# viniciusvidal2/slam-sensor-fusion

Hardware: AMD Instinct MI355X
Metric: scans_per_s_200k_scan_vs_10M_map (higher is better)
Workload: dtype f32 points / f64 accumulation

## Files before the change

### slam_sensor_fusion_amd/csrc/sf_icp.hip

```cpp
#include "sf_common.hpp"
#include "sf_nn.hpp"
#include "sf_tile.hpp"
#include "sf_order.hpp"
#include "sf_p2p.hpp"

#include <cfloat>
#include <cstdlib>
#include <cmath>
#include <vector>
#include <mutex>
#include <string>

namespace {

constexpr int BLK = 256;
constexpr int NREC_P2P = 17;
constexpr int NREC_PLANE = 30;
constexpr int REC_STRIDE = 32;

struct IcpState {
    double T[16];
    double rec[REC_STRIDE];
    double fitness, rmse, prev_fitness, prev_rmse;
    float last_error, err_pending;
// ... 799 lines not shown
        for (int k = 0; k < 12; ++k) P.T[k] = (float)st[b].T[k];
        return P;
    }
    __device__ __forceinline__ Point load(uint32_t o) const { return Point{x[o], y[o], z[o]}; }
    __device__ __forceinline__ uint32_t full_key(const Pose &P, const Point &p) const
    {
        const float qx = fmaf(P.T[0], p.x, fmaf(P.T[1], p.y, fmaf(P.T[2], p.z, P.T[3])));
        const float qy = fmaf(P.T[4], p.x, fmaf(P.T[5], p.y, fmaf(P.T[6], p.z, P.T[7])));
        const float qz = fmaf(P.T[8], p.x, fmaf(P.T[9], p.y, fmaf(P.T[10], p.z, P.T[11])));
        if (!(isfinite(qx) && isfinite(qy) && isfinite(qz))) return TILE_KEY_NONE;
        const int cx = (int)fminf(fmaxf(floorf((qx - g.org[0]) * g.inv_h), 0.0f), (float)(g.dim[0] - 1));
        const int cy = (int)fminf(fmaxf(floorf((qy - g.org[1]) * g.inv_h), 0.0f), (float)(g.dim[1] - 1));
        const int cz = (int)fminf(fmaxf(floorf((qz - g.org[2]) * g.inv_h), 0.0f), (float)(g.dim[2] - 1));
        return sf::tile_of_cell(tl, cx, cy, cz);
    }
    __device__ __forceinline__ uint32_t key(const Pose &P, const Point &p) const { return (full_key(P, p) >> (sf::ORD_KEY_BITS * digit)) & (uint32_t)(sf::ORD_BINS - 1); }
};

__global__ __launch_bounds__(sf::ORD_BLK) void k_order_hist_tile(sf::OrderSrc s, TileKeyFn kf, uint16_t *__restrict__ keys, uint32_t *__restrict__ counts)
{
    sf::order_hist_body(s, kf, keys, counts);
}

__global__ __launch_bounds__(256) void k_tile_keys(TileKeyFn kf, int64_t total, uint32_t *__restrict__ tkey)
{
    const int64_t o = (int64_t)blockIdx.x * 256 + threadIdx.x;
    if (o >= total) return;
    const int b = (int)(o / kf.n);
    tkey[o] = kf.full_key(kf.prepare(b), kf.load((uint32_t)o));
}

__global__ __launch_bounds__(256) void k_tile_starts(const uint32_t *__restrict__ tkey, int n, int batch, int ntiles, uint32_t *__restrict__ seg)
{
    const int64_t i = (int64_t)blockIdx.x * 256 + threadIdx.x;
    if (i >= (int64_t)(ntiles + 1) * batch) return;
    const uint32_t t = (uint32_t)(i / batch);
    const int b = (int)(i % batch);
    const uint32_t *k = tkey + (size_t)b * n;
    int lo = 0, hi = n;
    while (lo < hi) {
        const int mid = (lo + hi) >> 1;
        if (k[mid] < t) lo = mid + 1; else hi = mid;
    }
    seg[i] = (uint32_t)lo;
}

constexpr int TILE_STATS = 8;
#ifdef SF_PHASE_TRACE
__device__ unsigned long long g_tile_trace[sf::PH_SHARDS * sf::PH_SLOTS];
#define TT_MARK(i) do { if (wv == 0) { const unsigned long long n_ = __builtin_amdgcn_s_memtime(); tt_acc[i] += (unsigned)(n_ - tt_t); tt_t = n_; } } while (0)
#else
#define TT_MARK(i) do { } while (0)
#endif

template <int MODE>
__global__ __launch_bounds__(sf::TILE_BLK) void k_tile_search(SfGrid g, sf::SfTiles tl, const float *__restrict__ X0x, const float *__restrict__ X0y, const float *__restrict__ X0z,
                                                              int n, int batch, const IcpState *__restrict__ st, float thr, const uint32_t *__restrict__ seg,
                                                              float4 *__restrict__ qcache, int64_t cache_n, int reuse, unsigned long long *__restrict__ stats)
{
    const int per = ((int)gridDim.x) >> 3;
    const int tile = ((int)blockIdx.x & 7) * per + ((int)blockIdx.x >> 3);
    if (tile >= tl.ntiles) return;
    __shared__ sf::TileLds lds;
    __shared__ double Tm[sf::TILE_SCANS][12];
    __shared__ float mot[sf::TILE_SCANS];
    __shared__ int live[sf::TILE_SCANS];
    __shared__ uint32_t pre[sf::TILE_SCANS + 1], gofs[sf::TILE_SCANS];
    __shared__ unsigned int cnt[4];
    const int tid = (int)threadIdx.x, lane = tid & 63, wv = tid >> 6;
    const sf::TileRegion R = sf::tile_region(g, tl, (uint32_t)tile);
#ifdef SF_PHASE_TRACE
    unsigned tt_acc[8] = {0, 0, 0, 0, 0, 0, 0, 0};
    unsigned long long tt_t = __builtin_amdgcn_s_memtime();
#endif
    bool staged = false, fits = false;
    if (tid < 4) cnt[tid] = 0;
    float *ecache = reinterpret_cast<float *>(qcache + (size_t)cache_n);
    SfWindow nowin;
    nowin.kind = 0;
    for (int b0 = 0; b0 < batch; b0 += sf::TILE_SCANS) {
        __syncthreads();
        if (wv == 0) {
            const int b = b0 + lane;
            uint32_t s0 = 0, len = 0;
            if (b < batch && !st[b].done) {
                s0 = seg[(size_t)tile * batch + b];
                len = seg[(size_t)(tile + 1) * batch + b] - s0;
            }
            uint32_t v = len;
#pragma unroll
            for (int o = 1; o < 64; o <<= 1) {
                const uint32_t t = (uint32_t)__shfl_up((int)v, o);
                if (lane >= o) v += t;
            }
            pre[lane + 1] = v;
            if (lane == 0) pre[0] = 0;
            gofs[lane] = (uint32_t)((size_t)b * n + s0);
        }
        for (int i = tid; i < sf::TILE_SCANS * 12; i += sf::TILE_BLK) {
            const int b = b0 + i / 12;
            Tm[i / 12][i % 12] = b < batch ? st[b].T[i % 12] : 0.0;
        }
        if (tid < sf::TILE_SCANS) {
            const int b = b0 + tid;
            mot[tid] = b < batch ? (float)st[b].motion : 0.0f;
            live[tid] = (b < batch && reuse && st[b].cache_live != 0) ? 1 : 0;
        }
        __syncthreads();
        TT_MARK(0);
        const uint32_t total = pre[sf::TILE_SCANS];
        if (total == 0) continue;
        if (!staged) {
            fits = sf::tile_stage(g, R, &lds);
            staged = true;
            if (!fits && tid == 0 && stats) atomicAdd(&stats[4], 1ull);
        }
        TT_MARK(1);
        for (uint32_t i = (uint32_t)tid; i < total; i += sf::TILE_BLK) {
            int bl = 0;
#pragma unroll
            for (int step = 32; step > 0; step >>= 1) bl += (pre[bl + step] <= i) ? step : 0;
            const size_t o = (size_t)gofs[bl] + (size_t)(i - pre[bl]);
            const bool cache_live = live[bl] != 0;
            float4 c1 = make_float4(0.f, 0.f, 0.f, 0.f), c2 = c1;
            float e = 0.0f;
            if (cache_live) {
                c1 = qcache[o];
                if (MODE == 2) { c2 = qcache[(size_t)cache_n + o]; e = c2.w; }
                else e = ecache[o];
            }
            const double x0 = X0x[o], y0 = X0y[o], z0 = X0z[o];
            const double *T = Tm[bl];
            const double sx = T[0] * x0 + T[1] * y0 + T[2] * z0 + T[3];
            const double sy = T[4] * x0 + T[5] * y0 + T[6] * z0 + T[7];
            const double sz = T[8] * x0 + T[9] * y0 + T[10] * z0 + T[11];
            const float qx = (float)sx, qy = (float)sy, qz = (float)sz;
            const float m_now = mot[bl];
            sf::NNHit chit, seed;
            float4 tn;
            bool need = reuse_certificate(true, qx, qy, qz, thr, m_now, e, c1, c2, chit, tn, seed);
            if (!need) {
                if (!cache_live) {
                    if (MODE == 2) qcache[(size_t)cache_n + o] = make_float4(0.f, 0.f, 0.f, 0.f);
                    else ecache[o] = 0.0f;
                }
                continue;
            }
            sf::NNHit hit;
            hit.d2 = sf::search_start(thr);
            hit.j = -1;
            hit.px = hit.py = hit.pz = 0.0f;
            hit.lb2 = 3.0e38f;
            bool walk = g.n > 0;
            {
                const float ox = fmaxf(fmaxf(g.org[0] - qx, qx - (g.org[0] + (float)g.dim[0] * g.h)), 0.0f);
                const float oy = fmaxf(fmaxf(g.org[1] - qy, qy - (g.org[1] + (float)g.dim[1] * g.h)), 0.0f);
                const float oz = fmaxf(fmaxf(g.org[2] - qz, qz - (g.org[2] + (float)g.dim[2] * g.h)), 0.0f);
                const float gap = fmaxf(sqrtf(ox * ox + oy * oy + oz * oz) * 0.9995f - 1.0e-3f, 0.0f);
                if (gap * gap > thr) { hit.lb2 = gap * gap; walk = false; }
            }
            if (walk) {
                const sf::QueryGeo G = sf::query_geo(g, qx, qy, qz);
                int ring_from = 1;
                if (fits && sf::tile_serves(g, R, G)) {
                    bool more;
                    const sf::TileHit th = sf::tile_search(g, R, &lds, G, qx, qy, qz, thr, seed.d2, seed.j, &more);
                    hit.d2 = th.d2; hit.j = th.j; hit.lb2 = th.lb2;
                    if (th.loc >= 0) { const float4 p = lds.pts[th.loc]; hit.px = p.x; hit.py = p.y; hit.pz = p.z; }
                    else if (th.j >= 0) { hit.px = seed.px; hit.py = seed.py; hit.pz = seed.pz; }
                    ring_from = more ? 2 : 0;
                    if (stats) atomicAdd(&cnt[more ? 3 : 1], 1u);
                } else {
                    if (seed.j >= 0 && seed.d2 < thr) { hit.d2 = seed.d2; hit.j = seed.j; hit.px = seed.px; hit.py = seed.py; hit.pz = seed.pz; }
                    if (stats) atomicAdd(&cnt[2], 1u);
                }
                if (ring_from) {
                    sf::nn_rings<false>(g, nowin, qx, qy, qz, ring_from, hit);
                    hit.lb2 = 0.0f;
                }
            }
            if (stats) atomicAdd(&cnt[0], 1u);
            float4 nrm = make_float4(0.f, 0.f, 0.f, 0.f);
            if (MODE == 2 && hit.j >= 0) nrm = g.nrm[hit.j];
            const float en = fmaxf(sqrtf(hit.lb2) * 0.9999f + m_now * 0.999998f - 1.0e-6f, 1.0e-30f);
            qcache[o] = make_float4(hit.px, hit.py, hit.pz, __int_as_float(hit.j));
            if (MODE == 2) qcache[(size_t)cache_n + o] = make_float4(nrm.x, nrm.y, nrm.z, en);
            else ecache[o] = en;
        }
    }
    TT_MARK(2);
    __syncthreads();
    TT_MARK(3);
    if (stats && tid < 4 && cnt[tid]) atomicAdd(&stats[tid], (unsigned long long)cnt[tid]);
#ifdef SF_PHASE_TRACE
    if (tid == 0) {
        tt_acc[7] = 1;
        for (int i = 0; i < 8; ++i) atomicAdd(&g_tile_trace[(size_t)(blockIdx.x & (sf::PH_SHARDS - 1)) * sf::PH_SLOTS + i], (unsigned long long)tt_acc[i]);
    }
#endif
}

template <int MODE, int Q>
__global__ __launch_bounds__(BLK) void k_red_cached(const float *__restrict__ X0x, const float *__restrict__ X0y, const float *__restrict__ X0z, int n,
                                                    const IcpState *__restrict__ st, float thr, double *__restrict__ partials, int nblocks, const float4 *__restrict__ qcache,
                                                    int64_t cache_n)
{
    constexpr int NREC = MODE == 2 ? NREC_PLANE : NREC_P2P;
    const int L = blockIdx.y * gridDim.x + blockIdx.x;
    const int kk = L >> 3;
    const int b = kk % (int)gridDim.y;
    const int bx = (L & 7) * ((int)gridDim.x >> 3) + kk / (int)gridDim.y;
    if (bx >= nblocks) return;
    const IcpState *S = st + b;
    if (S->done) return;
    __shared__ double stage[BLK / 64][32];
    const int wv = threadIdx.x >> 6, lane = threadIdx.x & 63;
    LanePair P[Q];
#pragma unroll
    for (int u = 0; u < Q; ++u) {
        const int slot = bx * (BLK * Q) + u * BLK + (int)threadIdx.x;
        const QueryIn q = query_in<MODE, false>(X0x, X0y, X0z, n, b, S, 0.0f, 0.0f, nullptr, qcache, cache_n, true, slot, n);
        sf::NNHit hit;
// ... 1431 lines not shown
    int64_t fused_redone = 0;
    bool inject_timeout = false;
    int64_t fused_launches = 0;
    IcpState *h_pin = nullptr;
    size_t h_pin_cap = 0;
    bool use_graph = false;
    hipGraphExec_t graph_exec = nullptr;
    int64_t graph_captures = 0, graph_replays = 0;
    struct GraphKey {
        int mode = -1, iters = -1, batch = -1, window = -1, ordered = -1, reuse = -1, robust_kind = -1;
        int64_t n = -1;
        const void *map = nullptr;
        uint64_t map_generation = 0, epochs = 0;
        float max_corr = 0, accept = 0, eps = 0;
        double robust_k = 0;
        bool operator==(const GraphKey &o) const
        {
            return mode == o.mode && iters == o.iters && batch == o.batch && window == o.window && ordered == o.ordered && reuse == o.reuse && n == o.n && map == o.map &&
                   map_generation == o.map_generation && epochs == o.epochs && max_corr == o.max_corr && accept == o.accept && eps == o.eps &&
                   robust_kind == o.robust_kind && robust_k == o.robust_k;
        }
    } graph_key;
    struct Lane {
        sf::DevBuf X, qcache, Xq, qkeys, qkeys2, qidx, qidx2, corr, state, d_inits, partials, fz_state, fz_part, fz_cnt, fz_ids, fz_all, qtkey, tseg, tile_stats;
        hipGraphExec_t graph_exec = nullptr;
        GraphKey graph_key;
        std::vector<double> inits_uploaded;
        uint32_t d_inits_epoch = 0xffffffffu;
    } other;
    struct SrcSet {
        sf::DevBuf X0, X0r, stage, d_boxes, d_box_parts, n_dev;
        int64_t n = 0, n_cap = 0, plane = 0;
        int batch = 0, nblocks = 0, nblocks_nn = 0, qpl = 1;
        bool have_source = false, n_on_device = false;
    } other_src;
    int src_set = 0;
    hipEvent_t src_used[2] = {nullptr, nullptr}, src_ready = nullptr;
    bool src_used_rec[2] = {false, false};
    bool src_ahead = false;
    hipEvent_t started[2] = {nullptr, nullptr};
    bool started_rec[2] = {false, false};
    hipEvent_t unmarked_ev = nullptr;
    bool src_unmarked_use = false;
    struct LaneMeta {
        bool valid = false;
        int batch = 0, mode = 0;
        std::vector<double> inits;
// ... 16 lines not shown
    bool profiling = false;
    std::vector<hipEvent_t> ev;
    size_t ev_used = 0;
    int64_t prof_launches = 0;
    double prof_ms = 0;
    std::vector<float> prof_each;
    std::vector<int> ev_kind;
    std::vector<float> prof_phase[SF_PROF_KINDS];
    sf::DevBuf nn_stats;
    int freeze = 1;
    FreezeParams fz_prm{8.0f, 2.0e-5f, 3.0e-4f, 3};
    int fz_from = 5;
    bool fz_from_auto = true;
    int fz_fetches = 0;
    int fz_step = 0;
    sf::DevBuf fz_state, fz_part, fz_cnt, fz_ids, fz_all;
    int64_t nn_stats_used = 0;
    static constexpr int64_t NN_STATS_CAP = 1024;
    int robust_kind = SF_ROBUST_NONE;
    double robust_k = 0.0;
    int tile_mode = 0;
    bool tile_on = false;
    sf::SfTiles tiles{};
    sf::DevBuf qtkey, tseg, tile_stats;
};

namespace {

float *soa(sf::DevBuf &b, int64_t total, int axis) { return b.as<float>() + (size_t)axis * (size_t)total; }
const float *src(sf_icp *icp, int axis)
{
    if (icp->shard) return soa(icp->Xq, icp->own_total, axis);
    return soa(icp->ordered ? icp->Xq : icp->X0, icp->plane, axis);
}

int fused_capacity(sf_icp *icp, int mode, bool robust = false);

bool robust_on(const sf_icp *icp, int mode) { return mode == SF_ICP_P2PLANE && icp->robust_kind != SF_ROBUST_NONE; }
RobustArg robust_arg(const sf_icp *icp) { return RobustArg{icp->robust_kind, icp->robust_k}; }

constexpr int64_t ORDER_AUTO_MIN_QUERIES = 300000;

int order_key_shift(const SfGrid &g)
{
    const uint64_t ny_pad = ((uint64_t)g.dim[1] + ORDER_YBLK - 1) / ORDER_YBLK * ORDER_YBLK;
    const uint64_t ncell = (uint64_t)g.dim[0] * ny_pad * (uint64_t)g.dim[2];
    int cbits = 0;
// ... 33 lines not shown
        tc[0] = t2[0]; tc[1] = t2[1]; tc[2] = t2[2];
    }
    if (!fits_tables(tc)) return false;
    sf::SfTiles tl;
    int64_t nt = 1;
    for (int a = 0; a < 3; ++a) {
        tl.tc[a] = tc[a];
        tl.nt[a] = (g.dim[a] + tc[a] - 1) / tc[a];
        nt *= tl.nt[a];
    }
    if (nt >= (int64_t)TILE_KEY_NONE) return false;
    tl.ntiles = (int)nt;
    *out = tl;
    return true;
}

bool tile_wanted(const sf_icp *icp, int mode)
{
    if (icp->tile_mode == 0 || robust_on(icp, mode) || icp->shard || icp->map->window.kind != 0 || (mode != SF_ICP_P2PLANE && mode != SF_ICP_O3D_P2P)) return false;
    if (icp->qpl == 1) return false;
    return icp->tile_mode == 2 || icp->n * icp->batch >= TILE_AUTO_MIN_QUERIES;
}

bool tile_launch(const sf_icp *icp, int k) { return icp->tile_on && (!icp->reuse || k < VERIFY_FROM_SEARCH); }

constexpr int ORDER_LUT_BINS = (1 << ORDER_LUT_LOG2) + 1;
int order_lut_prepare(sf_icp *icp)
{
    if (!icp->order_lut_on || !icp->map || !icp->map->built) return SF_OK;
    const SfGrid &g = icp->map->grid;
    if (g.n <= 0 || (icp->order_lut.p && icp->order_lut_gen == icp->map->generation)) return SF_OK;
    const uint64_t ny_pad = ((uint64_t)g.dim[1] + ORDER_YBLK - 1) / ORDER_YBLK * ORDER_YBLK;
    const uint64_t span = (uint64_t)g.dim[0] * ny_pad * (uint64_t)g.dim[2];
    int cbits = 0;
    while (cbits < 63 && (1ull << cbits) < span) ++cbits;
    icp->order_lut_shift = std::max(0, cbits - ORDER_LUT_LOG2);
    const int nbins = (int)(span >> icp->order_lut_shift) + 1;
    SF_TRY(icp->order_lut.reserve(sizeof(uint32_t) * (size_t)ORDER_LUT_BINS + sizeof(uint16_t) * (size_t)ORDER_LUT_BINS));
    uint32_t *hist = icp->order_lut.as<uint32_t>();
    uint16_t *lut = reinterpret_cast<uint16_t *>(hist + ORDER_LUT_BINS);
    hipStream_t st = icp->ctx->stream;
    SF_HIP(hipMemsetAsync(hist, 0, sizeof(uint32_t) * (size_t)ORDER_LUT_BINS, st));
    hipLaunchKernelGGL(k_order_lut_hist, dim3(nblk(g.n)), dim3(256), 0, st, g, icp->order_lut_shift, hist);
    hipLaunchKernelGGL(k_order_lut_make, dim3(1), dim3(1024), 0, st, hist, nbins, (uint32_t)g.n, lut);
    SF_HIP(hipGetLastError());
    icp->order_lut_gen = icp->map->generation;
    return SF_OK;
// ... 54 lines not shown
            hipLaunchKernelGGL(sf::k_order_scan, dim3((unsigned)nseg), dim3(sf::ORD_BINS), 0, s, counts, src2.tiles);
            hipLaunchKernelGGL(k_order_scatter, grid, blk, 0, s, src2, keys, counts, ordered);
        }
    } else {
        hipLaunchKernelGGL(k_order_hist, grid, blk, 0, s, src, kf, keys, counts);
        hipLaunchKernelGGL(sf::k_order_scan, dim3((unsigned)nseg), dim3(sf::ORD_BINS), 0, s, counts, src.tiles);
        hipLaunchKernelGGL(k_order_scatter, grid, blk, 0, s, src, keys, counts, ordered);
    }
    const int64_t qplane = seg_off ? total : icp->plane;
    if (seg_off) {
        hipLaunchKernelGGL(k_order_gather, dim3(nblk(total, GATHER_TILE)), dim3(256), 0, s, icp->X0r.as<float4>(), ordered, total, 0, 0, 0, soa(icp->Xq, qplane, 0),
                           soa(icp->Xq, qplane, 1), soa(icp->Xq, qplane, 2));
    } else {
        const int gt = (int)std::max<int64_t>(1, sf::div_up(icp->n, GATHER_TILE));
        hipLaunchKernelGGL(k_order_gather, dim3(sf::order_grid(gt, nseg)), dim3(256), 0, s, icp->X0r.as<float4>(), ordered, total, (int)icp->n, gt, nseg,
                           soa(icp->Xq, qplane, 0), soa(icp->Xq, qplane, 1), soa(icp->Xq, qplane, 2));
    }
    if (icp->tile_on) {
        TileKeyFn tk;
        tk.g = g; tk.tl = icp->tiles;
        tk.x = soa(icp->Xq, qplane, 0); tk.y = soa(icp->Xq, qplane, 1); tk.z = soa(icp->Xq, qplane, 2);
        tk.st = kf.st; tk.n = (int)icp->n; tk.digit = 0;
        const int64_t rows = (int64_t)icp->tiles.ntiles + 1;
        SF_TRY(icp->qtkey.reserve(sizeof(uint32_t) * cap));
        SF_TRY(icp->tseg.reserve(sizeof(uint32_t) * (size_t)rows * (size_t)nseg));
        SF_TRY(icp->tile_stats.reserve(sizeof(unsigned long long) * TILE_STATS));
        SF_HIP(hipMemsetAsync(icp->tile_stats.p, 0, sizeof(unsigned long long) * TILE_STATS, s));
        hipLaunchKernelGGL(k_tile_keys, dim3(nblk(total)), dim3(256), 0, s, tk, total, icp->qtkey.as<uint32_t>());
        hipLaunchKernelGGL(k_tile_starts, dim3(nblk(rows * nseg)), dim3(256), 0, s, icp->qtkey.as<uint32_t>(), (int)icp->n, nseg, icp->tiles.ntiles, icp->tseg.as<uint32_t>());
    }
    SF_HIP(hipGetLastError());
    return SF_OK;
}

int order_queries(sf_icp *icp, int mode)
{
    const int64_t total = icp->n * icp->batch;
    const bool want = icp->order == SF_ORDER_CELL || (icp->order == SF_ORDER_AUTO && total >= ORDER_AUTO_MIN_QUERIES);
    icp->ordered = false;
    icp->tile_on = false;
    if (!want || total == 0 || icp->map->grid.n == 0 || icp->n_on_device) return SF_OK;
    icp->tile_on = tile_wanted(icp, mode) && tile_plan(icp->map->grid, &icp->tiles);
    SF_TRY(run_order_sort(icp, icp->batch, icp->n, total, nullptr, nullptr));
    icp->ordered = true;
    return SF_OK;
}

void raw_swap(sf::DevBuf &a, sf::DevBuf &b)
{
    std::swap(a.p, b.p);
    std::swap(a.cap, b.cap);
    std::swap(a.epoch, b.epoch);
// ... 150 lines not shown

void prof_collect(sf_icp *icp)
{
    for (size_t k = 0; k + 1 < icp->ev_used; k += 2) {
        float ms = 0;
        if (hipEventElapsedTime(&ms, icp->ev[k], icp->ev[k + 1]) != hipSuccess) continue;
        const int kind = k / 2 < icp->ev_kind.size() ? icp->ev_kind[k / 2] : SF_PROF_NN;
        if (kind == SF_PROF_NN) { icp->prof_ms += ms; icp->prof_launches += 1; icp->prof_each.push_back(ms); }
        else if (kind > 0 && kind < SF_PROF_KINDS) icp->prof_phase[kind].push_back(ms);
    }
    icp->ev_used = 0;
}

sf_icp::GraphKey graph_key_now(const sf_icp *icp, int mode)
{
    sf_icp::GraphKey k;
    k.mode = mode; k.iters = icp->prm.num_iters; k.batch = icp->batch; k.window = icp->map->window.kind; k.ordered = (int)icp->ordered | ((int)icp->tile_on << 1); k.reuse = (int)icp->reuse | (icp->freeze << 1) | (icp->fz_from << 3);
    k.n = (mode == SF_ICP_REF_CPP && icp->batch == 1) ? -icp->n_cap : icp->n;
    k.map = (const void *)icp->map;
    k.map_generation = icp->map->generation;
    k.robust_kind = robust_on(icp, mode) ? icp->robust_kind : SF_ROBUST_NONE; k.robust_k = robust_on(icp, mode) ? icp->robust_k : 0.0;
    k.max_corr = icp->prm.max_corr; k.accept = icp->prm.accept; k.eps = icp->prm.eps + icp->fz_prm.guard_scale * 1.0e-3f + icp->fz_prm.guard_min + icp->fz_prm.guard_max + (float)icp->fz_prm.max_tries;
    const sf::DevBuf *bufs[] = {&icp->X0, &icp->X0r, &icp->X, &icp->Xq, &icp->qcache, &icp->corr, &icp->state, &icp->partials, &icp->d_box, &icp->d_boxes, &icp->n_dev,
                                &icp->map->pts4, &icp->map->nrm4, &icp->map->cell_start, &icp->map->d_window, &icp->fz_state, &icp->fz_part, &icp->fz_cnt, &icp->fz_ids, &icp->fz_all, &icp->tseg, &icp->tile_stats};
    k.epochs = (uint64_t)icp->plane;
    for (const sf::DevBuf *b : bufs) k.epochs = (k.epochs * 1000003ull + b->epoch) * 1000003ull + (uint64_t)(uintptr_t)b->p;
    return k;
}

float o3d_thr(const sf_icp *icp) { return (float)((double)icp->prm.max_corr * (double)icp->prm.max_corr); }

template <int MODE>
void launch_nn_red(sf_icp *icp, bool sharded = false, bool one_per_lane = false)
{
    sf_map *m = icp->map;
    const int nb = sharded ? (one_per_lane ? icp->own_nblocks * icp->qpl : icp->own_nblocks) : (one_per_lane ? icp->nblocks : icp->nblocks_nn);
    const dim3 grid((unsigned)((nb + 7) & ~7), (unsigned)icp->batch), blk(BLK);
    const float *x = src(icp, 0), *y = src(icp, 1), *z = src(icp, 2);
    const IcpState *st = icp->state.as<IcpState>();
    double *part = icp->partials.as<double>();
    const float thr = o3d_thr(icp);
    hipStream_t s = icp->ctx->stream;
    ProfScope ps(icp);
    uint32_t *stats = nullptr;
    if (icp->profiling && icp->nn_stats.p && icp->nn_stats_used < sf_icp::NN_STATS_CAP) stats = icp->nn_stats.as<uint32_t>() + 2 * NN_STATS_SHARDS * icp->nn_stats_used++;
    const bool win = m->window.kind != 0;
    if (MODE == 2 && robust_on(icp, MODE)) {
// ... 5 lines not shown
        if (win && sharded) { if (q1) SF_LAUNCH_NNRED_ROB(true, true, 1); else SF_LAUNCH_NNRED_ROB(true, true, SF_WIDE_QPL); }
        else if (win) { if (q1) SF_LAUNCH_NNRED_ROB(true, false, 1); else SF_LAUNCH_NNRED_ROB(true, false, SF_WIDE_QPL); }
        else if (sharded) { if (q1) SF_LAUNCH_NNRED_ROB(false, true, 1); else SF_LAUNCH_NNRED_ROB(false, true, SF_WIDE_QPL); }
        else { if (q1) SF_LAUNCH_NNRED_ROB(false, false, 1); else SF_LAUNCH_NNRED_ROB(false, false, SF_WIDE_QPL); }
#undef SF_LAUNCH_NNRED_ROB
        return;
    }
#define SF_LAUNCH_NNRED_Q(W, S, QQ)                                                                                                                              \
    hipLaunchKernelGGL((k_nn_red<MODE, W, S, QQ>), grid, blk, 0, s, m->grid, m->window, x, y, z, (int)icp->n, st, thr, icp->xlo, icp->xhi, part, nb, \
                       icp->own_off.as<uint32_t>(), icp->reuse ? icp->qcache.as<float4>() : nullptr, icp->cache_n, stats)
#define SF_LAUNCH_NNRED(W, S)                                  \
    do {                                                       \
        if (icp->qpl == 1 || one_per_lane) SF_LAUNCH_NNRED_Q(W, S, 1); \
        else SF_LAUNCH_NNRED_Q(W, S, SF_WIDE_QPL);             \
    } while (0)
    if (win && sharded) SF_LAUNCH_NNRED(true, true);
    else if (win) SF_LAUNCH_NNRED(true, false);
    else if (sharded) SF_LAUNCH_NNRED(false, true);
    else SF_LAUNCH_NNRED(false, false);
#undef SF_LAUNCH_NNRED_Q
#undef SF_LAUNCH_NNRED
}

template <int MODE>
void launch_tile_search(sf_icp *icp, bool one_per_lane)
{
    sf_map *m = icp->map;
    const int nb = one_per_lane ? icp->nblocks : icp->nblocks_nn;
    const float *x = src(icp, 0), *y = src(icp, 1), *z = src(icp, 2);
    const IcpState *st = icp->state.as<IcpState>();
    const float thr = o3d_thr(icp);
    hipStream_t s = icp->ctx->stream;
    ProfScope ps(icp);
    unsigned long long *stats = icp->profiling ? icp->tile_stats.as<unsigned long long>() : nullptr;
    if (icp->profiling && icp->nn_stats.p && icp->nn_stats_used < sf_icp::NN_STATS_CAP) icp->nn_stats_used++;
    const unsigned tgrid = (unsigned)((icp->tiles.ntiles + 7) & ~7);
    hipLaunchKernelGGL((k_tile_search<MODE>), dim3(tgrid), dim3(sf::TILE_BLK), 0, s, m->grid, icp->tiles, x, y, z, (int)icp->n, icp->batch, st, thr, icp->tseg.as<uint32_t>(),
                       icp->qcache.as<float4>(), icp->cache_n, (int)icp->reuse, stats);
    const dim3 grid((unsigned)((nb + 7) & ~7), (unsigned)icp->batch), blk(BLK);
    if (icp->qpl == 1 || one_per_lane)
        hipLaunchKernelGGL((k_red_cached<MODE, 1>), grid, blk, 0, s, x, y, z, (int)icp->n, st, thr, icp->partials.as<double>(), nb, icp->qcache.as<float4>(), icp->cache_n);
    else
        hipLaunchKernelGGL((k_red_cached<MODE, SF_WIDE_QPL>), grid, blk, 0, s, x, y, z, (int)icp->n, st, thr, icp->partials.as<double>(), nb, icp->qcache.as<float4>(), icp->cache_n);
}

bool freeze_on(const sf_icp *icp, int mode)
{
    const int64_t queries = icp->shard ? icp->own_total : icp->n * icp->batch;
    const bool wanted = icp->freeze == 2 || (icp->freeze == 1 && queries >= FREEZE_AUTO_MIN_QUERIES);
    return mode == SF_ICP_P2PLANE && wanted && !robust_on(icp, mode) && icp->reuse && icp->qpl == SF_WIDE_QPL && icp->map->window.kind == 0 && icp->prm.num_iters > icp->fz_from + 1 &&
           icp->fz_from >= VERIFY_FROM_SEARCH;
}

int freeze_alloc(sf_icp *icp)
{
    const size_t rows = (size_t)icp->batch * (size_t)std::max(icp->nblocks_nn, icp->shard ? icp->own_nblocks : 0);
    SF_TRY(icp->fz_state.reserve(sizeof(FreezeState) * (size_t)icp->batch));
    SF_TRY(icp->fz_part.reserve(sizeof(double) * FZ_NMOM * rows));
    SF_TRY(icp->fz_cnt.reserve(sizeof(uint32_t) * rows));
    SF_TRY(icp->fz_ids.reserve(sizeof(uint16_t) * FZ_CAP * rows));
    SF_TRY(icp->fz_all.reserve(sizeof(uint32_t) * FZ_CAP * rows));
// ... 706 lines not shown
}

extern "C" int sf_icp_test_inject_barrier_timeout(sf_icp *icp)
{
    SF_CHECK(icp, SF_ERR_INVALID, "icp is NULL");
    icp->inject_timeout = true;
    return SF_OK;
}

extern "C" int sf_icp_use_graph(sf_icp *icp, int on)
{
    SF_CHECK(icp, SF_ERR_INVALID, "icp is NULL");
    icp->use_graph = on != 0;
    return SF_OK;
}

namespace {
void lane_flip(sf_icp *icp)
{
    sf_icp::Lane &o = icp->other;
    raw_swap(icp->X, o.X); raw_swap(icp->qcache, o.qcache); raw_swap(icp->Xq, o.Xq); raw_swap(icp->qkeys, o.qkeys); raw_swap(icp->qkeys2, o.qkeys2);
    raw_swap(icp->qidx, o.qidx); raw_swap(icp->qidx2, o.qidx2); raw_swap(icp->corr, o.corr); raw_swap(icp->state, o.state); raw_swap(icp->d_inits, o.d_inits);
    raw_swap(icp->partials, o.partials); raw_swap(icp->fz_state, o.fz_state); raw_swap(icp->fz_part, o.fz_part); raw_swap(icp->fz_cnt, o.fz_cnt);
    raw_swap(icp->fz_ids, o.fz_ids); raw_swap(icp->fz_all, o.fz_all); raw_swap(icp->qtkey, o.qtkey); raw_swap(icp->tseg, o.tseg); raw_swap(icp->tile_stats, o.tile_stats);
    std::swap(icp->graph_exec, o.graph_exec);
    std::swap(icp->graph_key, o.graph_key);
    std::swap(icp->inits_uploaded, o.inits_uploaded);
    std::swap(icp->d_inits_epoch, o.d_inits_epoch);
    std::swap(icp->meta, icp->other_meta);
    icp->lane ^= 1;
}

int lane_reserve(sf_icp *icp)
{
    const int batch = std::max(icp->batch, 1);
    SF_TRY(icp->state.reserve(sizeof(IcpState) * (size_t)batch));
    SF_TRY(icp->d_inits.reserve(sizeof(double) * 16 * (size_t)batch));
    SF_TRY(icp->partials.reserve(sizeof(double) * (size_t)REC_STRIDE * (size_t)std::max(icp->nblocks, 1) * (size_t)batch));
    return SF_OK;
}

struct LaneScope {
    sf_icp *icp;
    hipStream_t main = nullptr;
    bool piped = false;
    int rc = SF_OK;
    LaneScope(sf_icp *i, bool allowed) : icp(i)
// ... 550 lines not shown
```

### slam_sensor_fusion_amd/csrc/sf_tile.hpp

```cpp
#pragma once
#include "sf_nn.hpp"

namespace sf {

constexpr int TILE_HALO = 2;
constexpr int TILE_PCAP = 2304;
constexpr int TILE_RX_MAX = 16;
constexpr int TILE_ROWS_MAX = 160;
constexpr int TILE_BLK = 256;
constexpr int TILE_SCANS = 64;

struct SfTiles {
    int tc[3];
    int nt[3];
    int ntiles;
};

__device__ __forceinline__ uint32_t tile_of_cell(const SfTiles &tl, int cx, int cy, int cz)
{
    return ((uint32_t)(cz / tl.tc[2]) * (uint32_t)tl.nt[1] + (uint32_t)(cy / tl.tc[1])) * (uint32_t)tl.nt[0] + (uint32_t)(cx / tl.tc[0]);
}

struct TileRegion {
    int x0, y0, z0;
    int rx, ry, rz;
};

__device__ __forceinline__ TileRegion tile_region(const SfGrid &g, const SfTiles &tl, uint32_t tile)
{
    const int tx = (int)(tile % (uint32_t)tl.nt[0]), ty = (int)((tile / (uint32_t)tl.nt[0]) % (uint32_t)tl.nt[1]), tz = (int)(tile / ((uint32_t)tl.nt[0] * (uint32_t)tl.nt[1]));
    TileRegion R;
    R.x0 = max(tx * tl.tc[0] - TILE_HALO, 0);
    R.y0 = max(ty * tl.tc[1] - TILE_HALO, 0);
    R.z0 = max(tz * tl.tc[2] - TILE_HALO, 0);
    R.rx = min((tx + 1) * tl.tc[0] + TILE_HALO, g.dim[0]) - R.x0;
    R.ry = min((ty + 1) * tl.tc[1] + TILE_HALO, g.dim[1]) - R.y0;
    R.rz = min((tz + 1) * tl.tc[2] + TILE_HALO, g.dim[2]) - R.z0;
    return R;
}

struct TileLds {
    float4 pts[TILE_PCAP + 4];
    uint16_t lcs[TILE_ROWS_MAX * (TILE_RX_MAX + 1)];
    uint32_t row_a[TILE_ROWS_MAX];
    uint32_t row_base[TILE_ROWS_MAX + 1];
    int overflow;
};

__device__ __forceinline__ bool tile_stage(const SfGrid &g, const TileRegion &R, TileLds *L)
{
    const int tid = (int)threadIdx.x, lane = tid & 63, wv = tid >> 6;
    const int nrows = R.ry * R.rz, rxp = R.rx + 1;
    for (int r = tid; r < nrows; r += TILE_BLK) {
        const int y = R.y0 + r % R.ry, z = R.z0 + r / R.ry;
        const size_t c0 = ((size_t)z * g.dim[1] + y) * g.dim[0] + R.x0;
        const uint32_t a = g.cell_start[c0], e = g.cell_start[c0 + R.rx];
        L->row_a[r] = a;
        L->row_base[r + 1] = e - a;
    }
    __syncthreads();
    if (wv == 0) {
        uint32_t carry = 0;
        for (int r0 = 0; r0 < nrows; r0 += 64) {
            const int r = r0 + lane;
            uint32_t v = r < nrows ? L->row_base[r + 1] : 0u;
#pragma unroll
            for (int o = 1; o < 64; o <<= 1) {
                const uint32_t t = (uint32_t)__shfl_up((int)v, o);
                if (lane >= o) v += t;
            }
            if (r < nrows) L->row_base[r + 1] = carry + v;
            carry += (uint32_t)__shfl((int)v, 63);
        }
        if (lane == 0) {
            L->row_base[0] = 0;
            L->overflow = carry > (uint32_t)TILE_PCAP ? 1 : 0;
        }
    }
    __syncthreads();
    const bool fits = L->overflow == 0;
    if (fits) {
        const int sub = lane >> 4, sl = lane & 15;
        for (int r = wv * 4 + sub; r < nrows; r += 4 * (TILE_BLK / 64)) {
            const uint32_t a = L->row_a[r], base = L->row_base[r], len = L->row_base[r + 1] - base;
            for (uint32_t k = (uint32_t)sl; k < len; k += 16u) {
                const float4 p = g.pts[a + k];
                L->pts[base + k] = make_float4(p.x, p.y, p.z, __uint_as_float(a + k));
            }
        }
        for (int i = tid; i < nrows * rxp; i += TILE_BLK) {
            const int r = i / rxp, x = i - r * rxp;
            const int y = R.y0 + r % R.ry, z = R.z0 + r / R.ry;
            const size_t c0 = ((size_t)z * g.dim[1] + y) * g.dim[0] + R.x0;
            L->lcs[r * (TILE_RX_MAX + 1) + x] = (uint16_t)(L->row_base[r] + (g.cell_start[c0 + x] - L->row_a[r]));
        }
    }
    __syncthreads();
    return fits;
}

struct TileHit {
    float d2;
    int j;
    int loc;
    float lb2;
};

__device__ __forceinline__ void tile_chunk4(const TileLds *L, uint32_t a, uint32_t b, float qx, float qy, float qz, TileHit &hit)
{
    constexpr float BIG = 3.0e38f;
    const bool v1 = a + 1 < b, v2 = a + 2 < b, v3 = a + 3 < b;
    const float4 p0 = L->pts[a], p1 = L->pts[a + 1], p2 = L->pts[a + 2], p3 = L->pts[a + 3];
    const float d0 = l2_simple(qx, qy, qz, p0.x, p0.y, p0.z);
    const float d1 = v1 ? l2_simple(qx, qy, qz, p1.x, p1.y, p1.z) : BIG;
    const float d2 = v2 ? l2_simple(qx, qy, qz, p2.x, p2.y, p2.z) : BIG;
    const float d3 = v3 ? l2_simple(qx, qy, qz, p3.x, p3.y, p3.z) : BIG;
    const float m3 = min3f(d0, d1, d2);
// ... 81 lines not shown
```

Measured before the change: 18530.

## Split tile search spillover into compacted rest kernel and restage tiles in registers

```diff
diff --git a/slam_sensor_fusion_amd/csrc/sf_icp.hip b/slam_sensor_fusion_amd/csrc/sf_icp.hip
--- a/slam_sensor_fusion_amd/csrc/sf_icp.hip
+++ b/slam_sensor_fusion_amd/csrc/sf_icp.hip
@@ -845,27 +845,17 @@
     sf::order_hist_body(s, kf, keys, counts);
 }
 
-__global__ __launch_bounds__(256) void k_tile_keys(TileKeyFn kf, int64_t total, uint32_t *__restrict__ tkey)
+__global__ __launch_bounds__(256) void k_tile_starts(TileKeyFn kf, int64_t total, int ntiles, int batch, uint32_t *__restrict__ seg)
 {
     const int64_t o = (int64_t)blockIdx.x * 256 + threadIdx.x;
     if (o >= total) return;
-    const int b = (int)(o / kf.n);
-    tkey[o] = kf.full_key(kf.prepare(b), kf.load((uint32_t)o));
-}
-
-__global__ __launch_bounds__(256) void k_tile_starts(const uint32_t *__restrict__ tkey, int n, int batch, int ntiles, uint32_t *__restrict__ seg)
-{
-    const int64_t i = (int64_t)blockIdx.x * 256 + threadIdx.x;
-    if (i >= (int64_t)(ntiles + 1) * batch) return;
-    const uint32_t t = (uint32_t)(i / batch);
-    const int b = (int)(i % batch);
-    const uint32_t *k = tkey + (size_t)b * n;
-    int lo = 0, hi = n;
-    while (lo < hi) {
-        const int mid = (lo + hi) >> 1;
-        if (k[mid] < t) lo = mid + 1; else hi = mid;
-    }
-    seg[i] = (uint32_t)lo;
+    const int b = (int)(o / kf.n), p = (int)(o - (int64_t)b * kf.n);
+    const TileKeyFn::Pose P = kf.prepare(b);
+    const int k = (int)min(kf.full_key(P, kf.load((uint32_t)o)), (uint32_t)ntiles);
+    const int kp = p > 0 ? (int)min(kf.full_key(P, kf.load((uint32_t)(o - 1))), (uint32_t)ntiles) : -1;
+    for (int t = kp + 1; t <= k; ++t) seg[(size_t)t * batch + b] = (uint32_t)p;
+    if (p == kf.n - 1)
+        for (int t = k + 1; t <= ntiles; ++t) seg[(size_t)t * batch + b] = (uint32_t)kf.n;
 }
 
 constexpr int TILE_STATS = 8;
@@ -877,9 +867,23 @@
 #endif
 
 template <int MODE>
-__global__ __launch_bounds__(sf::TILE_BLK) void k_tile_search(SfGrid g, sf::SfTiles tl, const float *__restrict__ X0x, const float *__restrict__ X0y, const float *__restrict__ X0z,
+__device__ __forceinline__ void tile_store(const SfGrid &g, float4 *__restrict__ qcache, float *__restrict__ ecache, int64_t cache_n, size_t o, const sf::NNHit &hit, float m_now)
+{
+    float4 nrm = make_float4(0.f, 0.f, 0.f, 0.f);
+    if (MODE == 2 && hit.j >= 0) nrm = g.nrm[hit.j];
+    const float en = fmaxf(sqrtf(hit.lb2) * 0.9999f + m_now * 0.999998f - 1.0e-6f, 1.0e-30f);
+    qcache[o] = make_float4(hit.px, hit.py, hit.pz, __int_as_float(hit.j));
+    if (MODE == 2) qcache[(size_t)cache_n + o] = make_float4(nrm.x, nrm.y, nrm.z, en);
+    else ecache[o] = en;
+}
+
+#ifndef SF_TILE_MIN_WAVES
+#define SF_TILE_MIN_WAVES 6
+#endif
+template <int MODE>
+__global__ __launch_bounds__(sf::TILE_BLK, SF_TILE_MIN_WAVES) void k_tile_search(SfGrid g, sf::SfTiles tl, const float *__restrict__ X0x, const float *__restrict__ X0y, const float *__restrict__ X0z,
                                                               int n, int batch, const IcpState *__restrict__ st, float thr, const uint32_t *__restrict__ seg,
-                                                              float4 *__restrict__ qcache, int64_t cache_n, int reuse, unsigned long long *__restrict__ stats)
+                                                              float4 *__restrict__ qcache, int64_t cache_n, int reuse, uint32_t *__restrict__ work, unsigned long long *__restrict__ stats)
 {
     const int per = ((int)gridDim.x) >> 3;
     const int tile = ((int)blockIdx.x & 7) * per + ((int)blockIdx.x >> 3);
@@ -899,18 +903,23 @@
     bool staged = false, fits = false;
     if (tid < 4) cnt[tid] = 0;
     float *ecache = reinterpret_cast<float *>(qcache + (size_t)cache_n);
-    SfWindow nowin;
-    nowin.kind = 0;
+    {
+        uint32_t cs[sf::TILE_CPL];
+        sf::tile_cells_issue(g, R, cs);
+        sf::tile_cells_park(R, cs, &lds);
+    }
     for (int b0 = 0; b0 < batch; b0 += sf::TILE_SCANS) {
         __syncthreads();
         if (wv == 0) {
             const int b = b0 + lane;
-            uint32_t s0 = 0, len = 0;
-            if (b < batch && !st[b].done) {
+            uint32_t s0 = 0, s1 = 0;
+            bool on = false;
+            if (b < batch) {
+                on = !st[b].done;
                 s0 = seg[(size_t)tile * batch + b];
-                len = seg[(size_t)(tile + 1) * batch + b] - s0;
+                s1 = seg[(size_t)(tile + 1) * batch + b];
             }
-            uint32_t v = len;
+            uint32_t v = on ? s1 - s0 : 0u;
 #pragma unroll
             for (int o = 1; o < 64; o <<= 1) {
                 const uint32_t t = (uint32_t)__shfl_up((int)v, o);
@@ -939,76 +948,79 @@
             if (!fits && tid == 0 && stats) atomicAdd(&stats[4], 1ull);
         }
         TT_MARK(1);
-        for (uint32_t i = (uint32_t)tid; i < total; i += sf::TILE_BLK) {
-            int bl = 0;
-#pragma unroll
-            for (int step = 32; step > 0; step >>= 1) bl += (pre[bl + step] <= i) ? step : 0;
-            const size_t o = (size_t)gofs[bl] + (size_t)(i - pre[bl]);
-            const bool cache_live = live[bl] != 0;
-            float4 c1 = make_float4(0.f, 0.f, 0.f, 0.f), c2 = c1;
-            float e = 0.0f;
-            if (cache_live) {
-                c1 = qcache[o];
-                if (MODE == 2) { c2 = qcache[(size_t)cache_n + o]; e = c2.w; }
-                else e = ecache[o];
-            }
-            const double x0 = X0x[o], y0 = X0y[o], z0 = X0z[o];
-            const double *T = Tm[bl];
-            const double sx = T[0] * x0 + T[1] * y0 + T[2] * z0 + T[3];
-            const double sy = T[4] * x0 + T[5] * y0 + T[6] * z0 + T[7];
-            const double sz = T[8] * x0 + T[9] * y0 + T[10] * z0 + T[11];
-            const float qx = (float)sx, qy = (float)sy, qz = (float)sz;
-            const float m_now = mot[bl];
-            sf::NNHit chit, seed;
-            float4 tn;
-            bool need = reuse_certificate(true, qx, qy, qz, thr, m_now, e, c1, c2, chit, tn, seed);
-            if (!need) {
-                if (!cache_live) {
-                    if (MODE == 2) qcache[(size_t)cache_n + o] = make_float4(0.f, 0.f, 0.f, 0.f);
-                    else ecache[o] = 0.0f;
+        for (uint32_t base = (uint32_t)(wv * 64); base < total; base += sf::TILE_BLK) {
+            const uint32_t i = base + (uint32_t)lane;
+            bool rest = false;
+            uint32_t o = 0;
+            if (i < total) {
+                int bl = 0;
+#pragma unroll
+                for (int step = 32; step > 0; step >>= 1) bl += (pre[bl + step] <= i) ? step : 0;
+                o = gofs[bl] + (i - pre[bl]);
+                const bool cache_live = live[bl] != 0;
+                float4 c1 = make_float4(0.f, 0.f, 0.f, 0.f), c2 = c1;
+                float e = 0.0f;
+                if (cache_live) {
+                    c1 = qcache[o];
+                    if (MODE == 2) { c2 = qcache[(size_t)cache_n + o]; e = c2.w; }
+                    else e = ecache[o];
                 }
-                continue;
-            }
-            sf::NNHit hit;
-            hit.d2 = sf::search_start(thr);
-            hit.j = -1;
-            hit.px = hit.py = hit.pz = 0.0f;
-            hit.lb2 = 3.0e38f;
-            bool walk = g.n > 0;
-            {
-                const float ox = fmaxf(fmaxf(g.org[0] - qx, qx - (g.org[0] + (float)g.dim[0] * g.h)), 0.0f);
-                const float oy = fmaxf(fmaxf(g.org[1] - qy, qy - (g.org[1] + (float)g.dim[1] * g.h)), 0.0f);
-                const float oz = fmaxf(fmaxf(g.org[2] - qz, qz - (g.org[2] + (float)g.dim[2] * g.h)), 0.0f);
-                const float gap = fmaxf(sqrtf(ox * ox + oy * oy + oz * oz) * 0.9995f - 1.0e-3f, 0.0f);
-                if (gap * gap > thr) { hit.lb2 = gap * gap; walk = false; }
-            }
-            if (walk) {
-                const sf::QueryGeo G = sf::query_geo(g, qx, qy, qz);
-                int ring_from = 1;
-                if (fits && sf::tile_serves(g, R, G)) {
-                    bool more;
-                    const sf::TileHit th = sf::tile_search(g, R, &lds, G, qx, qy, qz, thr, seed.d2, seed.j, &more);
-                    hit.d2 = th.d2; hit.j = th.j; hit.lb2 = th.lb2;
-                    if (th.loc >= 0) { const float4 p = lds.pts[th.loc]; hit.px = p.x; hit.py = p.y; hit.pz = p.z; }
-                    else if (th.j >= 0) { hit.px = seed.px; hit.py = seed.py; hit.pz = seed.pz; }
-                    ring_from = more ? 2 : 0;
-                    if (stats) atomicAdd(&cnt[more ? 3 : 1], 1u);
+                const double x0 = X0x[o], y0 = X0y[o], z0 = X0z[o];
+                const double *T = Tm[bl];
+                const double sx = T[0] * x0 + T[1] * y0 + T[2] * z0 + T[3];
+                const double sy = T[4] * x0 + T[5] * y0 + T[6] * z0 + T[7];
+                const double sz = T[8] * x0 + T[9] * y0 + T[10] * z0 + T[11];
+                const float qx = (float)sx, qy = (float)sy, qz = (float)sz;
+                const float m_now = mot[bl];
+                sf::NNHit chit, seed;
+                float4 tn;
+                const bool need = reuse_certificate(true, qx, qy, qz, thr, m_now, e, c1, c2, chit, tn, seed);
+                if (!need) {
+                    if (!cache_live) {
+                        if (MODE == 2) qcache[(size_t)cache_n + o] = make_float4(0.f, 0.f, 0.f, 0.f);
+                        else ecache[o] = 0.0f;
+                    }
                 } else {
-                    if (seed.j >= 0 && seed.d2 < thr) { hit.d2 = seed.d2; hit.j = seed.j; hit.px = seed.px; hit.py = seed.py; hit.pz = seed.pz; }
-                    if (stats) atomicAdd(&cnt[2], 1u);
-                }
-                if (ring_from) {
-                    sf::nn_rings<false>(g, nowin, qx, qy, qz, ring_from, hit);
-                    hit.lb2 = 0.0f;
+                    sf::NNHit hit;
+                    hit.d2 = sf::search_start(thr);
+                    hit.j = -1;
+                    hit.px = hit.py = hit.pz = 0.0f;
+                    hit.lb2 = 3.0e38f;
+                    bool walk = g.n > 0;
+                    {
+                        const float ox = fmaxf(fmaxf(g.org[0] - qx, qx - (g.org[0] + (float)g.dim[0] * g.h)), 0.0f);
+                        const float oy = fmaxf(fmaxf(g.org[1] - qy, qy - (g.org[1] + (float)g.dim[1] * g.h)), 0.0f);
+                        const float oz = fmaxf(fmaxf(g.org[2] - qz, qz - (g.org[2] + (float)g.dim[2] * g.h)), 0.0f);
+                        const float gap = fmaxf(sqrtf(ox * ox + oy * oy + oz * oz) * 0.9995f - 1.0e-3f, 0.0f);
+                        if (gap * gap > thr) { hit.lb2 = gap * gap; walk = false; }
+                    }
+                    if (walk) {
+                        const sf::QueryGeo G = sf::query_geo(g, qx, qy, qz);
+                        if (fits && sf::tile_serves(g, R, G)) {
+                            bool more;
+                            const sf::TileHit th = sf::tile_search(g, R, &lds, G, qx, qy, qz, thr, seed.d2, seed.j, &more);
+                            rest = more;
+                            hit.d2 = th.d2; hit.j = th.j; hit.lb2 = th.lb2;
+                            if (th.loc >= 0) { const float4 p = lds.pts[th.loc]; hit.px = p.x; hit.py = p.y; hit.pz = p.z; }
+                            else if (th.j >= 0) { hit.px = seed.px; hit.py = seed.py; hit.pz = seed.pz; }
+                            if (stats) atomicAdd(&cnt[more ? 3 : 1], 1u);
+                        } else {
+                            rest = true;
+                            if (stats) atomicAdd(&cnt[2], 1u);
+                        }
+                    }
+                    if (stats) atomicAdd(&cnt[0], 1u);
+                    if (!rest) tile_store<MODE>(g, qcache, ecache, cache_n, o, hit, m_now);
                 }
             }
-            if (stats) atomicAdd(&cnt[0], 1u);
-            float4 nrm = make_float4(0.f, 0.f, 0.f, 0.f);
-            if (MODE == 2 && hit.j >= 0) nrm = g.nrm[hit.j];
-            const float en = fmaxf(sqrtf(hit.lb2) * 0.9999f + m_now * 0.999998f - 1.0e-6f, 1.0e-30f);
-            qcache[o] = make_float4(hit.px, hit.py, hit.pz, __int_as_float(hit.j));
-            if (MODE == 2) qcache[(size_t)cache_n + o] = make_float4(nrm.x, nrm.y, nrm.z, en);
-            else ecache[o] = en;
+            const unsigned long long m = __ballot(rest);
+            if (m) {
+                const int first = __ffsll((long long)m) - 1;
+                uint32_t w0 = 0;
+                if (lane == first) w0 = atomicAdd(work, (uint32_t)__popcll(m));
+                w0 = (uint32_t)__shfl((int)w0, first);
+                if (rest) work[1 + w0 + __builtin_amdgcn_mbcnt_hi((unsigned)(m >> 32), __builtin_amdgcn_mbcnt_lo((unsigned)m, 0u))] = o;
+            }
         }
     }
     TT_MARK(2);
@@ -1021,6 +1033,46 @@
         for (int i = 0; i < 8; ++i) atomicAdd(&g_tile_trace[(size_t)(blockIdx.x & (sf::PH_SHARDS - 1)) * sf::PH_SLOTS + i], (unsigned long long)tt_acc[i]);
     }
 #endif
+}
+
+template <int MODE>
+__global__ __launch_bounds__(256) void k_tile_rest(SfGrid g, const float *__restrict__ X0x, const float *__restrict__ X0y, const float *__restrict__ X0z, int n,
+                                                   const IcpState *__restrict__ st, float thr, float4 *__restrict__ qcache, int64_t cache_n, int reuse, const uint32_t *__restrict__ work)
+{
+    const uint32_t count = work[0];
+    float *ecache = reinterpret_cast<float *>(qcache + (size_t)cache_n);
+    SfWindow nowin;
+    nowin.kind = 0;
+    for (uint32_t k = blockIdx.x * 256 + threadIdx.x; k < count; k += gridDim.x * 256) {
+        const uint32_t o = work[1 + k];
+        const IcpState *S = st + o / (uint32_t)n;
+        float4 c1 = make_float4(0.f, 0.f, 0.f, 0.f), c2 = c1;
+        float e = 0.0f;
+        if (reuse && S->cache_live != 0) {
+            c1 = qcache[o];
+            if (MODE == 2) { c2 = qcache[(size_t)cache_n + o]; e = c2.w; }
+            else e = ecache[o];
+        }
+        const double x0 = X0x[o], y0 = X0y[o], z0 = X0z[o];
+        const double *T = S->T;
+        const double sx = T[0] * x0 + T[1] * y0 + T[2] * z0 + T[3];
+        const double sy = T[4] * x0 + T[5] * y0 + T[6] * z0 + T[7];
+        const double sz = T[8] * x0 + T[9] * y0 + T[10] * z0 + T[11];
+        const float qx = (float)sx, qy = (float)sy, qz = (float)sz;
+        const float m_now = (float)S->motion;
+        sf::NNHit chit, seed;
+        float4 tn;
+        reuse_certificate(true, qx, qy, qz, thr, m_now, e, c1, c2, chit, tn, seed);
+        sf::NNHit hit;
+        hit.d2 = sf::search_start(thr);
+        hit.j = -1;
+        hit.px = hit.py = hit.pz = 0.0f;
+        hit.lb2 = 3.0e38f;
+        if (seed.j >= 0 && seed.d2 < thr) { hit.d2 = seed.d2; hit.j = seed.j; hit.px = seed.px; hit.py = seed.py; hit.pz = seed.pz; }
+        sf::nn_rings<false>(g, nowin, qx, qy, qz, 1, hit);
+        hit.lb2 = 0.0f;
+        tile_store<MODE>(g, qcache, ecache, cache_n, o, hit, m_now);
+    }
 }
 
 template <int MODE, int Q>
@@ -2498,7 +2550,7 @@
         }
     } graph_key;
     struct Lane {
-        sf::DevBuf X, qcache, Xq, qkeys, qkeys2, qidx, qidx2, corr, state, d_inits, partials, fz_state, fz_part, fz_cnt, fz_ids, fz_all, qtkey, tseg, tile_stats;
+        sf::DevBuf X, qcache, Xq, qkeys, qkeys2, qidx, qidx2, corr, state, d_inits, partials, fz_state, fz_part, fz_cnt, fz_ids, fz_all, twork, tseg, tile_stats;
         hipGraphExec_t graph_exec = nullptr;
         GraphKey graph_key;
         std::vector<double> inits_uploaded;
@@ -2561,7 +2613,7 @@
     int tile_mode = 0;
     bool tile_on = false;
     sf::SfTiles tiles{};
-    sf::DevBuf qtkey, tseg, tile_stats;
+    sf::DevBuf twork, tseg, tile_stats;
 };
 
 namespace {
@@ -2641,7 +2693,14 @@
     return icp->tile_mode == 2 || icp->n * icp->batch >= TILE_AUTO_MIN_QUERIES;
 }
 
-bool tile_launch(const sf_icp *icp, int k) { return icp->tile_on && (!icp->reuse || k < VERIFY_FROM_SEARCH); }
+constexpr int TILE_LAUNCHES = 2;
+static_assert(TILE_LAUNCHES <= VERIFY_FROM_SEARCH, "the tile launches run one query per lane");
+bool tile_launch(const sf_icp *icp, int k)
+{
+    if (!icp->tile_on) return false;
+    if (icp->tile_mode == 2) return !icp->reuse || k < VERIFY_FROM_SEARCH;
+    return k < TILE_LAUNCHES;
+}
 
 constexpr int ORDER_LUT_BINS = (1 << ORDER_LUT_LOG2) + 1;
 int order_lut_prepare(sf_icp *icp)
@@ -2742,12 +2801,11 @@
         tk.x = soa(icp->Xq, qplane, 0); tk.y = soa(icp->Xq, qplane, 1); tk.z = soa(icp->Xq, qplane, 2);
         tk.st = kf.st; tk.n = (int)icp->n; tk.digit = 0;
         const int64_t rows = (int64_t)icp->tiles.ntiles + 1;
-        SF_TRY(icp->qtkey.reserve(sizeof(uint32_t) * cap));
+        SF_TRY(icp->twork.reserve(sizeof(uint32_t) * (cap + 1)));
         SF_TRY(icp->tseg.reserve(sizeof(uint32_t) * (size_t)rows * (size_t)nseg));
         SF_TRY(icp->tile_stats.reserve(sizeof(unsigned long long) * TILE_STATS));
         SF_HIP(hipMemsetAsync(icp->tile_stats.p, 0, sizeof(unsigned long long) * TILE_STATS, s));
-        hipLaunchKernelGGL(k_tile_keys, dim3(nblk(total)), dim3(256), 0, s, tk, total, icp->qtkey.as<uint32_t>());
-        hipLaunchKernelGGL(k_tile_starts, dim3(nblk(rows * nseg)), dim3(256), 0, s, icp->qtkey.as<uint32_t>(), (int)icp->n, nseg, icp->tiles.ntiles, icp->tseg.as<uint32_t>());
+        hipLaunchKernelGGL(k_tile_starts, dim3(nblk(total)), dim3(256), 0, s, tk, total, icp->tiles.ntiles, nseg, icp->tseg.as<uint32_t>());
     }
     SF_HIP(hipGetLastError());
     return SF_OK;
@@ -2944,7 +3002,7 @@
     k.robust_kind = robust_on(icp, mode) ? icp->robust_kind : SF_ROBUST_NONE; k.robust_k = robust_on(icp, mode) ? icp->robust_k : 0.0;
     k.max_corr = icp->prm.max_corr; k.accept = icp->prm.accept; k.eps = icp->prm.eps + icp->fz_prm.guard_scale * 1.0e-3f + icp->fz_prm.guard_min + icp->fz_prm.guard_max + (float)icp->fz_prm.max_tries;
     const sf::DevBuf *bufs[] = {&icp->X0, &icp->X0r, &icp->X, &icp->Xq, &icp->qcache, &icp->corr, &icp->state, &icp->partials, &icp->d_box, &icp->d_boxes, &icp->n_dev,
-                                &icp->map->pts4, &icp->map->nrm4, &icp->map->cell_start, &icp->map->d_window, &icp->fz_state, &icp->fz_part, &icp->fz_cnt, &icp->fz_ids, &icp->fz_all, &icp->tseg, &icp->tile_stats};
+                                &icp->map->pts4, &icp->map->nrm4, &icp->map->cell_start, &icp->map->d_window, &icp->fz_state, &icp->fz_part, &icp->fz_cnt, &icp->fz_ids, &icp->fz_all, &icp->tseg, &icp->twork, &icp->tile_stats};
     k.epochs = (uint64_t)icp->plane;
     for (const sf::DevBuf *b : bufs) k.epochs = (k.epochs * 1000003ull + b->epoch) * 1000003ull + (uint64_t)(uintptr_t)b->p;
     return k;
@@ -2996,6 +3054,7 @@
 #undef SF_LAUNCH_NNRED
 }
 
+constexpr int TILE_REST_BLOCKS = 512;
 template <int MODE>
 void launch_tile_search(sf_icp *icp, bool one_per_lane)
 {
@@ -3009,8 +3068,12 @@
     unsigned long long *stats = icp->profiling ? icp->tile_stats.as<unsigned long long>() : nullptr;
     if (icp->profiling && icp->nn_stats.p && icp->nn_stats_used < sf_icp::NN_STATS_CAP) icp->nn_stats_used++;
     const unsigned tgrid = (unsigned)((icp->tiles.ntiles + 7) & ~7);
+    uint32_t *work = icp->twork.as<uint32_t>();
+    const hipError_t e = hipMemsetAsync(work, 0, sizeof(uint32_t), s);
+    (void)e;
     hipLaunchKernelGGL((k_tile_search<MODE>), dim3(tgrid), dim3(sf::TILE_BLK), 0, s, m->grid, icp->tiles, x, y, z, (int)icp->n, icp->batch, st, thr, icp->tseg.as<uint32_t>(),
-                       icp->qcache.as<float4>(), icp->cache_n, (int)icp->reuse, stats);
+                       icp->qcache.as<float4>(), icp->cache_n, (int)icp->reuse, work, stats);
+    hipLaunchKernelGGL((k_tile_rest<MODE>), dim3(TILE_REST_BLOCKS), dim3(256), 0, s, m->grid, x, y, z, (int)icp->n, st, thr, icp->qcache.as<float4>(), icp->cache_n, (int)icp->reuse, work);
     const dim3 grid((unsigned)((nb + 7) & ~7), (unsigned)icp->batch), blk(BLK);
     if (icp->qpl == 1 || one_per_lane)
         hipLaunchKernelGGL((k_red_cached<MODE, 1>), grid, blk, 0, s, x, y, z, (int)icp->n, st, thr, icp->partials.as<double>(), nb, icp->qcache.as<float4>(), icp->cache_n);
@@ -3763,7 +3826,7 @@
     raw_swap(icp->X, o.X); raw_swap(icp->qcache, o.qcache); raw_swap(icp->Xq, o.Xq); raw_swap(icp->qkeys, o.qkeys); raw_swap(icp->qkeys2, o.qkeys2);
     raw_swap(icp->qidx, o.qidx); raw_swap(icp->qidx2, o.qidx2); raw_swap(icp->corr, o.corr); raw_swap(icp->state, o.state); raw_swap(icp->d_inits, o.d_inits);
     raw_swap(icp->partials, o.partials); raw_swap(icp->fz_state, o.fz_state); raw_swap(icp->fz_part, o.fz_part); raw_swap(icp->fz_cnt, o.fz_cnt);
-    raw_swap(icp->fz_ids, o.fz_ids); raw_swap(icp->fz_all, o.fz_all); raw_swap(icp->qtkey, o.qtkey); raw_swap(icp->tseg, o.tseg); raw_swap(icp->tile_stats, o.tile_stats);
+    raw_swap(icp->fz_ids, o.fz_ids); raw_swap(icp->fz_all, o.fz_all); raw_swap(icp->twork, o.twork); raw_swap(icp->tseg, o.tseg); raw_swap(icp->tile_stats, o.tile_stats);
     std::swap(icp->graph_exec, o.graph_exec);
     std::swap(icp->graph_key, o.graph_key);
     std::swap(icp->inits_uploaded, o.inits_uploaded);
diff --git a/slam_sensor_fusion_amd/csrc/sf_tile.hpp b/slam_sensor_fusion_amd/csrc/sf_tile.hpp
--- a/slam_sensor_fusion_amd/csrc/sf_tile.hpp
+++ b/slam_sensor_fusion_amd/csrc/sf_tile.hpp
@@ -7,8 +7,12 @@
 constexpr int TILE_PCAP = 2304;
 constexpr int TILE_RX_MAX = 16;
 constexpr int TILE_ROWS_MAX = 160;
-constexpr int TILE_BLK = 256;
+constexpr int TILE_BLK = 512;
 constexpr int TILE_SCANS = 64;
+constexpr int TILE_CELLS = TILE_ROWS_MAX * (TILE_RX_MAX + 1);
+constexpr int TILE_CPL = (TILE_CELLS + TILE_BLK - 1) / TILE_BLK;
+constexpr int TILE_PPL = (TILE_PCAP + TILE_BLK - 1) / TILE_BLK;
+static_assert(TILE_ROWS_MAX <= 256, "tile_row_of: an 8-step search over the row starts");
 
 struct SfTiles {
     int tc[3];
@@ -47,29 +51,59 @@
     int overflow;
 };
 
+__device__ __forceinline__ void tile_cells_issue(const SfGrid &g, const TileRegion &R, uint32_t (&cs)[TILE_CPL])
+{
+    const int tid = (int)threadIdx.x, rxp = R.rx + 1, ncs = R.ry * R.rz * rxp;
+#pragma unroll
+    for (int k = 0; k < TILE_CPL; ++k) {
+        const int i = tid + k * TILE_BLK;
+        cs[k] = 0u;
+        if (i < ncs) {
+            const int r = i / rxp, x = i - r * rxp;
+            const int y = R.y0 + r % R.ry, z = R.z0 + r / R.ry;
+            cs[k] = g.cell_start[((size_t)z * g.dim[1] + y) * g.dim[0] + R.x0 + x];
+        }
+    }
+}
+
+static_assert(TILE_CELLS <= 4 * TILE_PCAP, "the raw cell table is parked in the point area");
+__device__ __forceinline__ uint32_t *tile_cell_park(TileLds *L) { return reinterpret_cast<uint32_t *>(L->pts); }
+
+__device__ __forceinline__ void tile_cells_park(const TileRegion &R, const uint32_t (&cs)[TILE_CPL], TileLds *L)
+{
+    const int tid = (int)threadIdx.x, ncs = R.ry * R.rz * (R.rx + 1);
+    uint32_t *raw = tile_cell_park(L);
+#pragma unroll
+    for (int k = 0; k < TILE_CPL; ++k)
+        if (tid + k * TILE_BLK < ncs) raw[tid + k * TILE_BLK] = cs[k];
+}
+
+__device__ __forceinline__ int tile_row_of(const TileLds *L, int nrows, uint32_t i)
+{
+    int r = 0;
+#pragma unroll
+    for (int step = 128; step > 0; step >>= 1)
+        if (r + step < nrows && L->row_base[r + step] <= i) r += step;
+    return r;
+}
+
 __device__ __forceinline__ bool tile_stage(const SfGrid &g, const TileRegion &R, TileLds *L)
 {
     const int tid = (int)threadIdx.x, lane = tid & 63, wv = tid >> 6;
     const int nrows = R.ry * R.rz, rxp = R.rx + 1;
-    for (int r = tid; r < nrows; r += TILE_BLK) {
-        const int y = R.y0 + r % R.ry, z = R.z0 + r / R.ry;
-        const size_t c0 = ((size_t)z * g.dim[1] + y) * g.dim[0] + R.x0;
-        const uint32_t a = g.cell_start[c0], e = g.cell_start[c0 + R.rx];
-        L->row_a[r] = a;
-        L->row_base[r + 1] = e - a;
-    }
-    __syncthreads();
+    const uint32_t *raw = tile_cell_park(L);
     if (wv == 0) {
         uint32_t carry = 0;
         for (int r0 = 0; r0 < nrows; r0 += 64) {
             const int r = r0 + lane;
-            uint32_t v = r < nrows ? L->row_base[r + 1] : 0u;
+            uint32_t a = 0, v = 0;
+            if (r < nrows) { a = raw[r * rxp]; v = raw[r * rxp + R.rx] - a; }
 #pragma unroll
             for (int o = 1; o < 64; o <<= 1) {
                 const uint32_t t = (uint32_t)__shfl_up((int)v, o);
                 if (lane >= o) v += t;
             }
-            if (r < nrows) L->row_base[r + 1] = carry + v;
+            if (r < nrows) { L->row_a[r] = a; L->row_base[r + 1] = carry + v; }
             carry += (uint32_t)__shfl((int)v, 63);
         }
         if (lane == 0) {
@@ -79,20 +113,36 @@
     }
     __syncthreads();
     const bool fits = L->overflow == 0;
+    const uint32_t np = L->row_base[nrows];
+    float4 v[TILE_PPL];
+    uint32_t pos[TILE_PPL];
     if (fits) {
-        const int sub = lane >> 4, sl = lane & 15;
-        for (int r = wv * 4 + sub; r < nrows; r += 4 * (TILE_BLK / 64)) {
-            const uint32_t a = L->row_a[r], base = L->row_base[r], len = L->row_base[r + 1] - base;
-            for (uint32_t k = (uint32_t)sl; k < len; k += 16u) {
-                const float4 p = g.pts[a + k];
-                L->pts[base + k] = make_float4(p.x, p.y, p.z, __uint_as_float(a + k));
+#pragma unroll
+        for (int k = 0; k < TILE_PPL; ++k) {
+            const uint32_t i = (uint32_t)(tid + k * TILE_BLK);
+            pos[k] = 0u;
+            v[k] = make_float4(0.f, 0.f, 0.f, 0.f);
+            if (i < np) {
+                const int r = tile_row_of(L, nrows, i);
+                pos[k] = L->row_a[r] + (i - L->row_base[r]);
+                v[k] = g.pts[pos[k]];
             }
         }
-        for (int i = tid; i < nrows * rxp; i += TILE_BLK) {
-            const int r = i / rxp, x = i - r * rxp;
-            const int y = R.y0 + r % R.ry, z = R.z0 + r / R.ry;
-            const size_t c0 = ((size_t)z * g.dim[1] + y) * g.dim[0] + R.x0;
-            L->lcs[r * (TILE_RX_MAX + 1) + x] = (uint16_t)(L->row_base[r] + (g.cell_start[c0 + x] - L->row_a[r]));
+#pragma unroll
+        for (int k = 0; k < TILE_CPL; ++k) {
+            const int i = tid + k * TILE_BLK;
+            if (i < nrows * rxp) {
+                const int r = i / rxp, x = i - r * rxp;
+                L->lcs[r * (TILE_RX_MAX + 1) + x] = (uint16_t)(L->row_base[r] + (raw[i] - L->row_a[r]));
+            }
+        }
+    }
+    __syncthreads();
+    if (fits) {
+#pragma unroll
+        for (int k = 0; k < TILE_PPL; ++k) {
+            const uint32_t i = (uint32_t)(tid + k * TILE_BLK);
+            if (i < np) L->pts[i] = make_float4(v[k].x, v[k].y, v[k].z, __uint_as_float(pos[k]));
         }
     }
     __syncthreads();
```

After: 18440 (median of 2 runs). No clear change (-0.5%).
